# yixuan/LBFGSpp

Measured on AMD Instinct MI355X. Metric: L-BFGS iterations/sec at n=10^8, m=10; achieved HBM GB/s vs peak, higher is better.
Workload: dtype f64; 1 GPU; north-star: extended Rosenbrock n=100000000 m=10 f64 LineSearchMoreThuente, x0 from counter hash; n=100000000, m=10, history_full=True, fevals_total=111, apply_Hv_persistent_launches=82

## Files before the change

include/LBFGS.h:

```cpp
#ifndef LBFGSX_DROPIN_LBFGS_H
#define LBFGSX_DROPIN_LBFGS_H

#include <algorithm>
#include <cmath>
#include <cstdlib>
#include <cstring>
#include <exception>
#include <limits>
#include <stdexcept>
#include <string>
#include <thread>
#include <type_traits>
#include <vector>

#include "LBFGSpp/BKLDLT.h"
#include "LBFGSpp/DenseHessian.h"
#include "LBFGSpp/Device.h"
#include "LBFGSpp/Interop.h"
#include "LBFGSpp/GramSpace.h"
#include "LBFGSpp/LineSearchBacktracking.h"
#include "LBFGSpp/LineSearchBracketing.h"
#include "LBFGSpp/LineSearchMoreThuente.h"
#include "LBFGSpp/LineSearchNocedalWright.h"
#include "LBFGSpp/Param.h"
// ... 78 lines not shown
        if (gram)
        {
            gsh.direction(-1.0, gs_coef, gs_coef_g);
            detail::check(lbfgsx_gs_direction(c, gs_coef.data(), gs_coef_g, &dgd));
            if (m_reducer)
                m_reducer(&dgd, 1);
        }
        else
            detail::check(lbfgsx_apply_Hv(c, LBFGSX_VEC_G, m_dir_scale, &dgd));
        constexpr bool policy_defers =
            detail::takes_pending_dg<LineSearch<Scalar> >::value &&
            detail::has_device_line_search<LineSearch<Scalar>, detail::Evaluator<Scalar, Foo, HostVec>, LBFGSParam<Scalar>, Scalar>::value;
        const bool defer_dg = policy_defers && !gram && !m_reducer && !detail::is_compiled_objective<Scalar, Foo>::value &&
                              ev.builtin_id() >= 0;
        detail::check(lbfgsx_last_in_trial_request(c, defer_dg ? 1 : 0));
        Scalar dg = Scalar(dgd);
        Scalar step = Scalar(1) / m_gnorm;
        constexpr Scalar eps = std::numeric_limits<Scalar>::epsilon();

        int k = 1;
        for (;;)
        {
            detail::Range range_iteration("lbfgs:iteration");
            detail::check(lbfgsx_ls_begin(c));
            if (!gram)
                detail::check(lbfgsx_ls_post_in_trial(c, m_dir_scale));
            const Scalar step_max = m_param.max_step;
            ev.trial_written = false;
            try
            {
// ... 266 lines not shown
```

include/LBFGSpp/Interop.h:

```cpp
#ifndef LBFGSX_DROPIN_INTEROP_H
#define LBFGSX_DROPIN_INTEROP_H

#include <cstdint>
#include <type_traits>
#include <utility>
#include <vector>

#if !defined(LBFGSX_NO_EIGEN) && defined(__has_include)
#if __has_include(<Eigen/Core>)
#include <Eigen/Core>
#define LBFGSX_HAVE_EIGEN 1
#endif
#endif

#include "DenseHessian.h"

namespace LBFGSpp {
namespace detail {

#ifdef LBFGSX_HAVE_EIGEN
template <typename Scalar>
using ResultVector = Eigen::Matrix<Scalar, Eigen::Dynamic, 1>;
template <typename Scalar>
using ResultMatrix = Eigen::Matrix<Scalar, Eigen::Dynamic, Eigen::Dynamic>;
// ... 17 lines not shown

template <typename Policy, typename Ev, typename Param, typename Scalar, typename = void>
struct has_device_line_search : std::false_type {};
template <typename Policy, typename Ev, typename Param, typename Scalar>
struct has_device_line_search<Policy, Ev, Param, Scalar,
                              std::void_t<decltype(Policy::LineSearch(std::declval<Ev&>(), std::declval<const Param&>(),
                                                                      std::declval<const Scalar&>(), std::declval<Scalar&>(),
                                                                      std::declval<Scalar&>(), std::declval<Scalar&>()))> >
    : std::true_type {};

template <typename Policy, typename = void>
struct takes_pending_dg : std::false_type {};
template <typename Policy>
struct takes_pending_dg<Policy, std::enable_if_t<Policy::takes_pending_dg> > : std::true_type {};

template <typename Scalar, typename Ev, typename HostVec>
struct HostObjective
{
    Ev& ev;
    Scalar operator()(const HostVec& x, HostVec& grad) { return ev.eval_host_point(x, grad); }
};

template <typename Scalar, typename Policy, typename HostVec, typename Ev, typename Param>
inline void run_line_search(Ev& ev, const Param& param, const Scalar& step_max, Scalar& step, Scalar& fx, Scalar& dg)
{
    if constexpr (has_device_line_search<Policy, Ev, Param, Scalar>::value)
        Policy::LineSearch(ev, param, step_max, step, fx, dg);
    else
    {
        const std::int64_t n = ev.state().size();
// ... 26 lines not shown
```

include/LBFGSpp/LineSearchMoreThuente.h:

```cpp
#ifndef LBFGSX_DROPIN_LS_MORE_THUENTE_H
#define LBFGSX_DROPIN_LS_MORE_THUENTE_H

#include <algorithm>
#include <cmath>
#include <limits>
#include <stdexcept>

#include "HostEval.h"
#include "Param.h"

namespace LBFGSpp {

template <typename Scalar>
class LineSearchMoreThuente
{
    struct Sample
    {
        Scalar t, f, g;
    };

    static Scalar quad_fgf(const Sample& p, Scalar qt, Scalar fq)
    {
        const Scalar h = qt - p.t;
        const Scalar w = Scalar(0.5) * h * p.g / (p.f - fq + h * p.g);
// ... 206 lines not shown
                }
            }
            m_step = next;
            if (++m_it >= m_max_it)
            {
                m_step = m_lo.t;
                m_fx = m_f_best;
                m_dg = m_g_best;
                return DONE_LO;
            }
            return TRIAL;
        }
    };

    static constexpr bool takes_pending_dg = true;

    template <typename Eval, typename SolverParam>
    static void LineSearch(Eval& ev, const SolverParam& param, const Scalar& step_max, Scalar& step, Scalar& fx,
                           Scalar& dg)
    {
        Machine mt;
        bool have_first = false;
        if constexpr (detail::has_dg_pending<Eval>::value)
        {
            if (ev.dg_pending)
            {
                ev.dg_pending = false;
                mt.start_step(param, step_max, step, fx);
                Scalar f1 = fx, g1 = dg, dg0 = dg;
                have_first = ev.first_trial(mt.step(), f1, g1, dg0);
// ... 46 lines not shown
```

include/lbfgsx.h:

```cpp
#ifndef LBFGSX_H
#define LBFGSX_H

#include <stddef.h>
#include <stdint.h>

#ifdef __cplusplus
extern "C" {
#endif

typedef struct lbfgsx_ctx lbfgsx_ctx;

enum { LBFGSX_F64 = 0, LBFGSX_F32 = 1 };
enum { LBFGSX_OBJ_NONE = -1, LBFGSX_OBJ_DIAG_QUAD = 0, LBFGSX_OBJ_EXT_ROSENBROCK = 1,
       LBFGSX_OBJ_BOUND = 64  };
enum
{
    LBFGSX_OK = 0,
    LBFGSX_E_INVALID = -1,
    LBFGSX_E_LOGIC = -2,
    LBFGSX_E_RUNTIME = -3,
    LBFGSX_E_HIP = -4,
    LBFGSX_E_NOGPU = -5,
    LBFGSX_E_USER = -6
};
// ... 48 lines not shown
int lbfgsx_trial(lbfgsx_ctx* c, int objective, double step, double* fx, double* dg);
int lbfgsx_trial_point(lbfgsx_ctx* c, double step);
int lbfgsx_trial_dg(lbfgsx_ctx* c, double* dg);
int lbfgsx_ls_keep_trial_as_lo(lbfgsx_ctx* c);
int lbfgsx_ls_end(lbfgsx_ctx* c, int use_lo);
int lbfgsx_post_linesearch(lbfgsx_ctx* c, double* gnorm2, double* xnorm2, double* sy, double* yy);
int lbfgsx_commit_correction(lbfgsx_ctx* c);
int lbfgsx_post_linesearch_spec(lbfgsx_ctx* c, double a, double* gnorm2, double* xnorm2, double* sy, double* yy);
int lbfgsx_spec_counts(const lbfgsx_ctx* c, int64_t out[3]);
int lbfgsx_ls_post_in_trial(lbfgsx_ctx* c, double a);
int lbfgsx_post_in_trial_counts(const lbfgsx_ctx* c, int64_t out[4]);
int lbfgsx_last_in_trial_request(lbfgsx_ctx* c, int on);
int lbfgsx_apply_Hv_pending(lbfgsx_ctx* c, int v_which, double a, double* dg, int* pending);
int lbfgsx_trial_first(lbfgsx_ctx* c, int objective, double step, double* fx, double* dg, double* dg_init);
int lbfgsx_last_in_trial_counts(const lbfgsx_ctx* c, int64_t out[4]);
typedef struct lbfgsx_objective lbfgsx_objective;
int lbfgsx_objective_compile(lbfgsx_objective** out, int dtype, int K, const char* body, char* log, size_t log_len);
void lbfgsx_objective_destroy(lbfgsx_objective* obj);
long long lbfgsx_objective_source(int dtype, int K, const char* body, char* out, size_t len);
int lbfgsx_objective_info(const lbfgsx_objective* obj, long long out[8]);
int lbfgsx_objective_K(const lbfgsx_objective* obj);
int lbfgsx_objective_dtype(const lbfgsx_objective* obj);
int lbfgsx_objective_bind(lbfgsx_ctx* c, const lbfgsx_objective* obj, const void* const p[4], const double cs[8], int* id);
int lbfgsx_objective_upload(lbfgsx_ctx* c, int slot, const void* host, void** dev);
int lbfgsx_objective_bound(const lbfgsx_ctx* c, const void* p[4]);
enum { LBFGSX_FORM_TERM = 0, LBFGSX_FORM_CHAIN = 1, LBFGSX_FORM_GRID = 2, LBFGSX_FORM_GRAPH = 3, LBFGSX_FORM_MESH = 4, LBFGSX_FORM_LINEAR = 5,
       LBFGSX_FORM_LINEAR_MULTI = 6, LBFGSX_FORM_DENSE = 7, LBFGSX_FORM_LINEAR_GRAPH = 8, LBFGSX_FORM_VOLUME = 9,
       LBFGSX_FORM_GRID_PERIODIC = 10, LBFGSX_FORM_VOLUME_PERIODIC = 11, LBFGSX_FORM_GRID_FIELD = 12 };
int lbfgsx_objective_compile_chain(lbfgsx_objective** out, int dtype, int K, const char* body, char* log, size_t log_len);
long long lbfgsx_objective_source_chain(int dtype, int K, const char* body, char* out, size_t len);
// ... 277 lines not shown
```

lbfgspp_amd/_lib.py:

```python
import ctypes as C
import os

HERE = os.path.dirname(os.path.abspath(__file__))

F64, F32 = 0, 1
OBJ_DIAG_QUAD, OBJ_EXT_ROSENBROCK = 0, 1
OBJ_BOUND = 64
LS_NOCEDAL_WRIGHT, LS_MORE_THUENTE, LS_BACKTRACKING, LS_BRACKETING = 0, 1, 2, 3
ALGO_LBFGS, ALGO_LBFGSB = 0, 1
RECURSION_VECTOR, RECURSION_GRAM_SPACE, RECURSION_GRAM_SPACE_F32H = 0, 1, 2
FLAG_BOUNDED = 1
(VEC_X, VEC_G, VEC_XP, VEC_GP, VEC_D, VEC_XT, VEC_GT, VEC_A, VEC_B, VEC_LB, VEC_UB, VEC_XCP) = range(12)
E_INVALID, E_LOGIC, E_RUNTIME, E_HIP, E_NOGPU, E_USER = -1, -2, -3, -4, -5, -6


class Params(C.Structure):
    _fields_ = [("m", C.c_int), ("epsilon", C.c_double), ("epsilon_rel", C.c_double), ("past", C.c_int),
                ("delta", C.c_double), ("max_iterations", C.c_int), ("linesearch", C.c_int),
                ("max_linesearch", C.c_int), ("min_step", C.c_double), ("max_step", C.c_double),
                ("ftol", C.c_double), ("wolfe", C.c_double), ("max_submin", C.c_int)]


class Result(C.Structure):
    _fields_ = [("niter", C.c_int), ("nfev", C.c_int), ("fx", C.c_double), ("gnorm", C.c_double),
# ... 85 lines not shown
    sig(core, "lbfgsx_timing_enable", i32, vp, i32)
    sig(core, "lbfgsx_timing_read", i32, vp, pd, C.POINTER(i64), pd, C.POINTER(i64))
    sig(core, "lbfgsx_stream_probe", i32, vp, i32, pd, pd)
    sig(core, "lbfgsx_selftest_reduce", i32, vp, i32, i32, i32, pd)
    sig(core, "lbfgsx_post_linesearch_spec", i32, vp, dbl, pd, pd, pd, pd)
    sig(core, "lbfgsx_rccl_allgather_records", i32, C.POINTER(i32), i32, vp, i64, i64, C.POINTER(vp))
    sig(core, "lbfgsx_device_download", i32, i32, vp, i64, vp)
    sig(core, "lbfgsx_device_free", None, i32, vp)
    sig(core, "lbfgsx_spec_counts", i32, vp, C.POINTER(i64 * 3))
    sig(core, "lbfgsx_ls_post_in_trial", i32, vp, dbl)
    sig(core, "lbfgsx_post_in_trial_counts", i32, vp, C.POINTER(i64 * 4))
    sig(core, "lbfgsx_last_in_trial_request", i32, vp, i32)
    sig(core, "lbfgsx_apply_Hv_pending", i32, vp, i32, dbl, pd, C.POINTER(i32))
    sig(core, "lbfgsx_trial_first", i32, vp, i32, dbl, pd, pd, pd)
    sig(core, "lbfgsx_last_in_trial_counts", i32, vp, C.POINTER(i64 * 4))
    sig(core, "lbfgsx_counters", i32, C.POINTER(i64 * 3), i32)
    sig(core, "lbfgsx_counters_ex", i32, C.POINTER(i64 * 8), i32)
    sig(core, "lbfgsx_poll_counts", i32, vp, C.POINTER(i64 * 2))
    sig(core, "lbfgsx_poll_counts_ex", i32, vp, C.POINTER(i64 * 4))
    sig(core, "lbfgsx_b_compact_vec_counts", i32, C.POINTER(i64 * 4), i32)
    sig(core, "lbfgsx_b_reserve", i32, vp)
    sig(core, "lbfgsx_device", i32, vp)
    sig(core, "lbfgsx_persist_counts", i32, vp, C.POINTER(i64 * 4))
    sig(core, "lbfgsx_debug_persist_fault", i32, vp)

    sig(sol, "lbfgsx_solver_create", i32, C.POINTER(vp), i32, i32, i32, C.POINTER(Params), i32)
    sig(sol, "lbfgsx_solver_create_error", C.c_char_p)
    sig(sol, "lbfgsx_solver_destroy", None, vp)
    sig(sol, "lbfgsx_solver_prepare", i32, vp, i64)
    sig(sol, "lbfgsx_solver_ctx", vp, vp)
# ... 180 lines not shown
```

lbfgspp_amd/csrc/ctx.hpp:

```cpp
#pragma once
#include <hip/hip_runtime.h>
#include <stdint.h>

#include <atomic>
#include <chrono>
#include <string>
#include <vector>

#include "../../include/lbfgsx.h"
#include "last_step.hpp"
#include "reduce.cuh"

struct lbfgsx_ctx;
namespace lbfgsx {

void set_error(const std::string& msg);

#define LBFGSX_HIP(expr)                                                                      \
    do                                                                                        \
    {                                                                                         \
        hipError_t e_ = (expr);                                                               \
        if (e_ != hipSuccess)                                                                 \
        {                                                                                     \
            lbfgsx::set_error(std::string(#expr) + ": " + hipGetErrorString(e_) + " [" + __FILE__ + ":" + std::to_string(__LINE__) + "]");            \
            return LBFGSX_E_HIP;                                                              \
// ... 177 lines not shown
    int spec_cur = 0;
    double spec_a = 0.0, spec_dg = 0.0;
    int64_t spec_launches = 0, spec_used = 0, spec_rejected = 0;
    bool post_in_trial = true;
    bool pt_armed = false;
    double pt_a = 0.0;
    int ls_trials = 0;
    bool ls_first_ok = false;
    bool pt_valid = false;
    int pt_buf = -1, pt_xp = -1;
    double pt_r[4] = {0, 0, 0, 0};
    int64_t pt_issued = 0, pt_accepted = 0;
    int64_t from_g_launches = 0;
    lbfgsx::LastStep last;
    bool pt_builtin = false;

    const struct lbfgsx_objective* term = nullptr;
    void* term_fn[8] = {nullptr, nullptr, nullptr, nullptr, nullptr, nullptr, nullptr, nullptr};
    const void* term_p[4] = {nullptr, nullptr, nullptr, nullptr};
    double term_c[8] = {0, 0, 0, 0, 0, 0, 0, 0};
    int term_np = 0;
    int term_form = 0;
    int64_t term_rows = 0, term_cols = 0;
    int64_t term_slabs = 0;
    int term_periodic = 0;
    void* term_own[4] = {nullptr, nullptr, nullptr, nullptr};
    int64_t term_own_count[4] = {0, 0, 0, 0};
    int64_t graph_E = 0;
    void* graph_off = nullptr;
    void* graph_inc = nullptr;
// ... 121 lines not shown
```

lbfgspp_amd/csrc/lbfgs_kernels.cuh:

```cuda
#pragma once
#include "reduce.cuh"

namespace lbfgsx {

enum { OBJ_DIAG_QUAD = 0, OBJ_EXT_ROSENBROCK = 1 };

template <class T>
struct ObjQuad
{
    const T* a;
    const T* b;
    template <class A>
    __device__ __forceinline__ void pack(int64_t vi, const Pack<T>& x, Pack<T>& g, A& fx) const
    {
        const Pack<T> pa = ldv(a, vi), pb = ldv(b, vi);
#pragma unroll
        for (int k = 0; k < Vec16<T>::W; k++)
        {
            const T r = pa.e[k] * x.e[k] - pb.e[k];
            g.e[k] = pa.e[k] * r;
            fx.add(r * r);
        }
    }
    __device__ __forceinline__ T finish(T sum) const { return T(0.5) * sum; }
// ... 86 lines not shown
    T* dot0;
};

template <class T>
struct TrialLast
{
    const T* snew;
    const T* num;
    const T* num2;
    const T* den;
    T* dot0_keep;
    T* dg_slot;
    T* dout;
};

template <class T, class OBJ, bool POST, bool LAST = false>
__device__ __forceinline__ void trial_pass(const T* __restrict__ xp, const T* __restrict__ d, T step, T* __restrict__ x,
                                           T* __restrict__ g, int64_t n, const OBJ& obj, const RedWs& ws,
                                           T* __restrict__ out, int rev, const TrialPost<T>& tp,
                                           const TrialLast<T>& tl = TrialLast<T>())
{
    typedef typename AccOf<T>::type A;
    constexpr int W = Vec16<T>::W;
    constexpr int U = 4;
    constexpr bool SETTLE = LAST && !POST;
    constexpr int NRED = POST ? (LAST ? 8 : 7) : 2;
    A acc[NRED];
    T coef = T(0);
    if (LAST)
        coef = *tl.num / *tl.den - *tl.num2 / *tl.den;
    const int64_t nv = n / W;
    const int64_t tile = int64_t(kBlock) * U;
    const int64_t top = ((nv + tile - 1) / tile - 1) * tile;
    for (int64_t t0 = int64_t(blockIdx.x) * tile; t0 < nv; t0 += int64_t(gridDim.x) * tile)
    {
        const int64_t base = (rev ? top - t0 : t0) + threadIdx.x;
        Pack<T> pxp[U], pd[U], pgp[POST ? U : 1], psn[LAST ? U : 1];
#pragma unroll
        for (int u = 0; u < U; u++)
            if (base + u * kBlock < nv)
            {
// ... 5 lines not shown
                    pgp[POST ? u : 0] = ldv(tp.gp, base + u * kBlock);
            }
#pragma unroll
        for (int u = 0; u < U; u++)
        {
            const int64_t vi = base + u * kBlock;
            if (vi < nv)
            {
                Pack<T> px, pg;
                if (LAST)
                {
#pragma unroll
                    for (int k = 0; k < W; k++)
                    {
                        pd[u].e[k] = pd[u].e[k] + coef * psn[LAST ? u : 0].e[k];
                        if (POST)
                            acc[POST && LAST ? 7 : 0].add_prod(pgp[POST ? u : 0].e[k], pd[u].e[k]);
                    }
                    if (SETTLE)
                        stv(tl.dout, vi, pd[u]);
                }
#pragma unroll
                for (int k = 0; k < W; k++)
                    px.e[k] = pxp[u].e[k] + step * pd[u].e[k];
                obj.pack(vi, px, pg, acc[0]);
                stv(x, vi, px);
                stv(g, vi, pg);
#pragma unroll
                for (int k = 0; k < W; k++)
                    acc[1].add_prod(pg.e[k], pd[u].e[k]);
                if (POST)
                {
// ... 14 lines not shown
                    stv(tp.y, vi, py);
                }
            }
        }
    }
    if (blockIdx.x == 0 && threadIdx.x == 0)
    {
        auto dir = [&](int64_t i) { return LAST ? d[i] + coef * tl.snew[i] : d[i]; };
        for (int64_t i = nv * W; i < n; i++)
            x[i] = xp[i] + step * dir(i);
        for (int64_t i = nv * W; i < n; i++)
        {
            const T di = dir(i);
            obj.tail(i, n, x, g, acc[0]);
            acc[1].add_prod(g[i], di);
            if (POST && LAST)
                acc[POST && LAST ? 7 : 0].add_prod(tp.gp[i], di);
            if (SETTLE)
                tl.dout[i] = di;
        }
        if (POST)
            for (int64_t i = nv * W; i < n; i++)
            {
                const T si = x[i] - xp[i], yi = g[i] - tp.gp[i], q0 = tp.a * g[i];
                tp.s[i] = si;
                tp.y[i] = yi;
                acc[POST ? 2 : 0].add_prod(g[i], g[i]);
                acc[POST ? 3 : 0].add_prod(x[i], x[i]);
                acc[POST ? 4 : 0].add_prod(si, yi);
                acc[POST ? 5 : 0].add_prod(yi, yi);
                acc[POST ? 6 : 0].add_prod(si, q0);
            }
    }
    if (grid_reduce<NRED>(acc, ws) && threadIdx.x == 0)
    {
        out[0] = obj.finish(T(acc[0].value()));
        out[1] = T(acc[1].value());
        if (POST)
        {
            const T sy = T(acc[POST ? 4 : 0].value()), yy = T(acc[POST ? 5 : 0].value());
            out[2] = T(acc[POST ? 2 : 0].value());
            out[3] = T(acc[POST ? 3 : 0].value());
            out[4] = sy;
            out[5] = yy;
            if (LAST)
            {
                const T dgd = T(acc[LAST ? 7 : 0].value());
                out[6] = dgd;
                *tl.dg_slot = dgd;
                *tl.dot0_keep = *tl.num;
            }
            *tp.ys_slot = sy;
            *tp.theta_slot = yy / sy;
            *tp.dot0 = T(acc[POST ? 6 : 0].value());
        }
        ws_signal(ws);
    }
}

template <class T, class OBJ>
__global__ void __launch_bounds__(kBlock) k_trial(const T* __restrict__ xp, const T* __restrict__ d, T step,
                                                  T* __restrict__ x, T* __restrict__ g, int64_t n, OBJ obj,
// ... 10 lines not shown
}
template <class T, class OBJ>
__global__ void __launch_bounds__(kBlock, 4) k_trial_last(const T* __restrict__ xp, const T* __restrict__ q, T step,
                                                       T* __restrict__ x, T* __restrict__ g, int64_t n, OBJ obj,
                                                       RedWs ws, T* __restrict__ out, int rev, TrialPost<T> tp,
                                                       TrialLast<T> tl)
{
    trial_pass<T, OBJ, true, true>(xp, q, step, x, g, n, obj, ws, out, rev, tp, tl);
}
template <class T, class OBJ>
__global__ void __launch_bounds__(kBlock) k_trial_settle(const T* __restrict__ xp, const T* q, T step, T* __restrict__ x,
                                                         T* __restrict__ g, int64_t n, OBJ obj, RedWs ws,
                                                         T* __restrict__ out, int rev, TrialLast<T> tl)
{
    trial_pass<T, OBJ, false, true>(xp, q, step, x, g, n, obj, ws, out, rev, TrialPost<T>(), tl);
}

template <class T>
__global__ void __launch_bounds__(kBlock) k_axpy_point(const T* __restrict__ xp, const T* __restrict__ d, T step,
                                                       T* __restrict__ x, int64_t n)
{
    constexpr int W = Vec16<T>::W;
    const int64_t nv = n / W;
    const int64_t stride = int64_t(gridDim.x) * kBlock;
    for (int64_t vi = int64_t(blockIdx.x) * kBlock + threadIdx.x; vi < nv; vi += stride)
    {
        const Pack<T> pxp = ldv(xp, vi), pd = ldv(d, vi);
        Pack<T> px;
#pragma unroll
        for (int k = 0; k < W; k++)
// ... 968 lines not shown
```

lbfgspp_amd/csrc/lbfgsx.hip:

```cpp
#include <dlfcn.h>

#include <algorithm>
#include <atomic>
#include <cmath>
#include <chrono>
#include <string>
#include <vector>
#include <utility>
#include <cstdio>
#include <cstdlib>
#include <cstring>
#include <limits>
#include <mutex>

#include "ctx.hpp"
#include "lbfgs_kernels.cuh"
#include "launch_args.hpp"

namespace lbfgsx {

static std::atomic<int> g_live[64];
Counters& counters()
{
    static Counters g;
// ... 365 lines not shown
        if (n < min_n)
            c->persist = false;
    }
    if (const char* e = getenv("LBFGSX_PERSIST"))
        c->persist = atoi(e) != 0 && c->persist;
    if (const char* e = getenv("LBFGSX_MEET"))
        c->meet_all = std::strcmp(e, "last") != 0;
    if (const char* e = getenv("LBFGSX_PERSIST_POLL"))
        c->fast_persist_out = atoi(e) != 0;
    if (const char* e = getenv("LBFGSX_FUSE_POST"))
        c->fuse_post = atoi(e) != 0;
    if (const char* e = getenv("LBFGSX_POST_IN_TRIAL"))
        c->post_in_trial = atoi(e) != 0;
    if (const char* e = getenv("LBFGSX_LAST_IN_TRIAL"))
        c->last.enabled = atoi(e) != 0;
    {
        int occ = 0;
        hipDeviceProp_t prop;
        LBFGSX_HIP(hipGetDeviceProperties(&prop, device));
        if (dtype == LBFGSX_F64)
            (void) hipOccupancyMaxActiveBlocksPerMultiprocessor(&occ, k_twoloop_persist<double, true, true>, kHvThreads, 0);
        else
            (void) hipOccupancyMaxActiveBlocksPerMultiprocessor(&occ, k_twoloop_persist<float, true, true>, kHvThreads, 0);
        c->persist_grid = occ * prop.multiProcessorCount;
        c->gen_words = 16 + size_t(10) * size_t(c->persist_grid) * 4;
        LBFGSX_HIP(hipMalloc(reinterpret_cast<void**>(&c->gen_dev), c->gen_words * sizeof(unsigned)));
        LBFGSX_HIP(hipMemset(c->gen_dev, 0, c->gen_words * sizeof(unsigned)));
    }
    const size_t vbytes = size_t(c->ld) * c->esz;
    for (int k = 0; k < 3; k++)
// ... 660 lines not shown
        const T* g = P<T>(c->gb[c->cur]);
        LBFGSX_LAUNCH((k_dot<T>), dim3(grid), dim3(kBlock), 0, c->stream, g, g, P<T>(c->xb[c->cur]), c->n, c->ws,
                           c->out_slot<T>());
        int rc = fetch_scalars<T>(c, c->sl.out(0), 2, r);
        if (rc)
            return rc;
    });
    if (gnorm2) *gnorm2 = r[0];
    if (xnorm2) *xnorm2 = r[1];
    return LBFGSX_OK;
}

int lbfgsx_ls_begin(lbfgsx_ctx* c)
{
    c->st_valid = false;
    c->pt_valid = c->pt_armed = false;
    c->ls_trials = 0;
    c->xp = c->cur;
    c->lo = c->xp;
    c->trial = (c->xp + 1) % 3;
    return LBFGSX_OK;
}

}
template <class T, class OBJ>
static int trial_t(lbfgsx_ctx* c, OBJ obj, T step, double* out2)
{
    const lbfgsx::TrialLaunch<T> a = lbfgsx::trial_launch<T>(c, step, sizeof(OBJ) >= 2 * sizeof(void*) ? 2 : 0);
    LBFGSX_LAUNCH((k_trial<T, OBJ>), dim3(a.grid), dim3(kBlock), 0, c->stream, a.xp, a.d, a.step, a.x, a.g, a.n, obj, a.ws,
                       a.out, a.rev);
    LBFGSX_HIP(hipGetLastError());
    return fetch_scalars<T>(c, c->sl.out(0), 2, out2);
}
template <class T>
static lbfgsx::TrialPost<T> trial_post_args(lbfgsx_ctx* c)
{
    T* sc = P<T>(c->sc);
    return {P<T>(c->gb[c->xp]), P<T>(c->col(c->S, c->spare)), P<T>(c->col(c->Y, c->spare)), T(c->pt_a),
            sc + c->sl.ys(c->spare), sc + c->sl.theta(c->spare), sc + c->sl.dot(0)};
}
static void trial_post_done(lbfgsx_ctx* c, const double* out6)
{
    c->pending = false;
    c->pt_valid = true;
    c->pt_buf = c->trial;
    c->pt_xp = c->xp;
    for (int i = 0; i < 4; i++)
        c->pt_r[i] = out6[2 + i];
    c->pt_issued++;
}
template <class T, class OBJ>
static int trial_post_t(lbfgsx_ctx* c, OBJ obj, T step, double* out2)
{
    const lbfgsx::TrialLaunch<T> a = lbfgsx::trial_launch<T>(c, step, sizeof(OBJ) >= 2 * sizeof(void*) ? 2 : 0);
    const lbfgsx::TrialPost<T> tp = trial_post_args<T>(c);
    LBFGSX_LAUNCH((k_trial_post<T, OBJ>), dim3(a.grid), dim3(kBlock), 0, c->stream, a.xp, a.d, a.step, a.x, a.g, a.n, obj,
                       a.ws, a.out, a.rev, tp);
    LBFGSX_HIP(hipGetLastError());
    double r[6];
    const int rc = fetch_scalars<T>(c, c->sl.out(0), 6, r);
    if (rc)
        return rc;
    out2[0] = r[0];
    out2[1] = r[1];
    trial_post_done(c, r);
    c->pt_builtin = true;
    return LBFGSX_OK;
}
template <class T, class OBJ>
static int trial_last_t(lbfgsx_ctx* c, OBJ obj, T step, double* out3)
{
    const lbfgsx::LastStep& ls = c->last;
    if (ls.col == c->spare)
    {
        set_error("lbfgsx_trial: the newest history column is the spare column");
        return LBFGSX_E_LOGIC;
    }
    c->tl_step++;
    const lbfgsx::TrialLaunch<T> a = lbfgsx::trial_launch<T>(c, step, (sizeof(OBJ) >= 2 * sizeof(void*) ? 2 : 0) + 1);
    const lbfgsx::TrialPost<T> tp = trial_post_args<T>(c);
// ... 29 lines not shown
    T* sc = P<T>(c->sc);
    const lbfgsx::TrialLast<T> tl = {static_cast<const T*>(c->col(c->S, ls.col)), sc + c->sl.dot(2 * c->m + 1),
                                     sc + c->sl.dot(2 * ls.cn - 1), sc + c->sl.ys(ls.col), nullptr, nullptr, P<T>(c->d)};
    EventPair ev;
    int rc = last_time_begin(c, ev);
    if (rc)
        return rc;
    LBFGSX_LAUNCH((k_trial_settle<T, OBJ>), dim3(a.grid), dim3(kBlock), 0, c->stream, a.xp, a.d, a.step, a.x, a.g, a.n, obj,
                       a.ws, a.out, a.rev, tl);
    LBFGSX_HIP(hipGetLastError());
    if ((rc = last_time_end(c, ev)))
        return rc;
    (void) c->last.settle([](const lbfgsx::LastStep&) { return 0; });
    return fetch_scalars<T>(c, c->sl.out(0), 2, out2);
}
template <class T>
static int trial_post_term_t(lbfgsx_ctx* c, T step, double* out2)
{
    lbfgsx::TrialLaunch<T> a = lbfgsx::trial_launch<T>(c, step, c->term_np);
    lbfgsx::BoundArgs<T> obj(c);
    lbfgsx::TrialPost<T> tp = trial_post_args<T>(c);
    void* params[] = {&a.xp, &a.d, &a.step, &a.x, &a.g, &a.n, obj.ptr, &a.ws, &a.out, &a.rev, &tp};
    int rc = lbfgsx::jit_launch(c, lbfgsx::JIT_K_TRIAL_POST, a.grid, params);
    if (rc)
        return rc;
    double r[6];
    rc = fetch_scalars<T>(c, c->sl.out(0), 6, r);
    if (rc)
        return rc;
    out2[0] = r[0];
    out2[1] = r[1];
    trial_post_done(c, r);
    c->pt_builtin = false;
    return LBFGSX_OK;
}
template <class T>
static int trial_term_t(lbfgsx_ctx* c, T step, double* out2)
{
    lbfgsx::TrialLaunch<T> a = lbfgsx::trial_launch<T>(c, step, c->term_np);
    lbfgsx::BoundArgs<T> obj(c);
    lbfgsx::objective_model_add<T>(c, 2);
    void* params[] = {&a.xp, &a.d, &a.step, &a.x, &a.g, &a.n, obj.ptr, &a.ws, &a.out, &a.rev};
    int rc = lbfgsx::linear_pre_trial<T>(c, obj, a.xp, a.d, a.step);
    if (rc)
        return rc;
    rc = lbfgsx::jit_launch(c, lbfgsx::JIT_K_TRIAL, lbfgsx::linear_col_grid(c, a.grid), params);
    if (rc)
// ... 2 lines not shown
}
extern "C" {

int lbfgsx_trial(lbfgsx_ctx* c, int objective, double step, double* fx, double* dg)
{
    return lbfgsx_trial_first(c, objective, step, fx, dg, nullptr);
}

int lbfgsx_trial_first(lbfgsx_ctx* c, int objective, double step, double* fx, double* dg, double* dg_init)
{
    lbfgsx::DeviceGuard dev_guard_(c->device);
    c->spec_valid = false;
    double r[3];
    int rc = LBFGSX_E_INVALID;
    const bool builtin = objective == LBFGSX_OBJ_DIAG_QUAD || objective == LBFGSX_OBJ_EXT_ROSENBROCK;
    const bool last = c->last.fusable(c->pt_armed && c->ls_trials == 0, builtin, dg_init != nullptr, c->xp) && !c->st_valid;
    const int last_cn = c->last.cn;
    const bool settle_here = !last && c->last.pending && c->last.taken && builtin && !c->st_valid && c->xp == c->last.g;
    if (!last && !settle_here)
        LBFGSX_SETTLE(c);
    const bool owed = c->last.pay() && dg_init && !last;
    if (dg_init)
        *dg_init = std::numeric_limits<double>::quiet_NaN();
    if (c->st_valid)
    {
        c->st_valid = false;
        bool same = objective == c->st_obj && c->xp == c->st_xp && c->trial == c->st_trial;
        DISPATCH_T(c, { same = same && T(step) == T(c->st_step); });
        if (same)
        {
            c->st_hits++;
            c->ls_trials++;
            c->tl_step++;
            if (fx) *fx = c->st_f;
            if (dg) *dg = c->st_dg;
            return LBFGSX_OK;
        }
        c->st_cooldown = 4;
    }
    const bool post = c->pt_armed && c->ls_trials == 0 &&
                      (objective == LBFGSX_OBJ_DIAG_QUAD || objective == LBFGSX_OBJ_EXT_ROSENBROCK ||
                       (lbfgsx::term_bound(c, objective) && c->term_fn[lbfgsx::JIT_K_TRIAL_POST] != nullptr));
    c->ls_trials++;
    c->pt_valid = false;
    DISPATCH_T(c, {
        if (objective == LBFGSX_OBJ_DIAG_QUAD)
            rc = last          ? trial_last_t<T>(c, ObjQuad<T>{P<T>(c->a), P<T>(c->b)}, T(step), r)
                 : settle_here ? trial_settle_t<T>(c, ObjQuad<T>{P<T>(c->a), P<T>(c->b)}, T(step), r)
                 : post        ? trial_post_t<T>(c, ObjQuad<T>{P<T>(c->a), P<T>(c->b)}, T(step), r)
                               : trial_t<T>(c, ObjQuad<T>{P<T>(c->a), P<T>(c->b)}, T(step), r);
        else if (objective == LBFGSX_OBJ_EXT_ROSENBROCK)
            rc = last          ? trial_last_t<T>(c, ObjRosen<T>{}, T(step), r)
                 : settle_here ? trial_settle_t<T>(c, ObjRosen<T>{}, T(step), r)
                 : post        ? trial_post_t<T>(c, ObjRosen<T>{}, T(step), r)
                               : trial_t<T>(c, ObjRosen<T>{}, T(step), r);
        else if (lbfgsx::term_bound(c, objective))
            rc = post ? trial_post_term_t<T>(c, T(step), r) : trial_term_t<T>(c, T(step), r);
        else
            set_error("lbfgsx_trial: unknown objective");
        if (!rc && owed)
            rc = fetch_scalars<T>(c, c->sl.dot(2 * last_cn), 1, dg_init);
    });
    if (rc)
        return rc;
    if (fx) *fx = r[0];
    if (dg) *dg = r[1];
    if (last) *dg_init = r[2];
    return LBFGSX_OK;
}

int lbfgsx_trial_point(lbfgsx_ctx* c, double step)
{
// ... 203 lines not shown
        LBFGSX_HIP(hipMemsetAsync(c->ws.ticket, 0, sizeof(unsigned), c->stream));
        c->gen_count = 0;
        persist_timed_out(c);
        if (c->timing && !c->ev_hv.empty())
        {
            (void) hipEventDestroy(c->ev_hv.back().a);
            (void) hipEventDestroy(c->ev_hv.back().b);
            c->ev_hv.pop_back();
            c->persist_steps_timed -= 2 * cn + 1;
            c->fused_timed -= fused;
        }
        return 1;
    }
    c->persist_launches++;
    c->spec_launches++;
    c->from_g_launches += from_g ? 1 : 0;
    c->persist_backoff = 8;
    if (hflags[1] == 1)
    {
        c->spec_valid = true;
        c->spec_version = c->phys_version + 1;
        c->spec_cur = c->cur;
        c->spec_a = double(a);
        c->spec_dg = dgv;
        if (defer)
        {
            c->spec_dg = std::numeric_limits<double>::quiet_NaN();
            c->last.defer(cn, pa.pcol[0], c->cur);
        }
    }
    else
// ... 11 lines not shown
    return LBFGSX_OK;
}
extern "C" {

int lbfgsx_post_linesearch_spec(lbfgsx_ctx* c, double a, double* gnorm2, double* xnorm2, double* sy, double* yy)
{
    lbfgsx::DeviceGuard dev_guard_(c->device);
    if (c->gs_f32h)
        return lbfgsx_post_linesearch(c, gnorm2, xnorm2, sy, yy);
    double r[4];
    int rc = 1;
    c->spec_valid = false;
    if (c->pt_valid && c->cur == c->pt_buf && c->xp == c->pt_xp)
    {
        c->pt_valid = false;
        c->pt_accepted++;
        for (int i = 0; i < 4; i++)
            r[i] = c->pt_r[i];
        c->pend_sy = r[2];
        c->pend_yy = r[3];
        c->pending = true;
        bool usable = false;
        DISPATCH_T(c, { usable = a == c->pt_a && T(r[2]) > std::numeric_limits<T>::epsilon() * T(r[3]); });
        if (usable)
        {
            DISPATCH_T(c, { rc = post_spec_t<T>(c, T(a), r, true); });
            if (rc != LBFGSX_OK && rc != 1)
                return rc;
        }
        if (gnorm2) *gnorm2 = r[0];
        if (xnorm2) *xnorm2 = r[1];
// ... 12 lines not shown
    c->pending = true;
    if (gnorm2) *gnorm2 = r[0];
    if (xnorm2) *xnorm2 = r[1];
    if (sy) *sy = r[2];
    if (yy) *yy = r[3];
    return LBFGSX_OK;
}

int lbfgsx_ls_post_in_trial(lbfgsx_ctx* c, double a)
{
    if (!c)
        return LBFGSX_E_INVALID;
    c->pt_a = a;
    c->pt_armed = c->post_in_trial && c->ls_first_ok && c->ncorr > 0 && !c->gs_f32h && c->ls_trials == 0 &&
                  c->shard_off == 0 && c->n_global == c->n;
    return LBFGSX_OK;
}

int lbfgsx_post_in_trial_counts(const lbfgsx_ctx* c, int64_t out[4])
{
    if (!c || !out)
        return LBFGSX_E_INVALID;
    out[0] = c->pt_issued;
    out[1] = c->pt_accepted;
    out[2] = c->from_g_launches;
    out[3] = c->post_in_trial ? 1 : 0;
    return LBFGSX_OK;
}

int lbfgsx_last_in_trial_request(lbfgsx_ctx* c, int on)
{
    if (!c)
        return LBFGSX_E_INVALID;
    c->last.requested = on != 0 && !c->bstate;
    return LBFGSX_OK;
}

int lbfgsx_last_in_trial_counts(const lbfgsx_ctx* c, int64_t out[4])
{
    if (!c || !out)
        return LBFGSX_E_INVALID;
// ... 326 lines not shown
```

Measured before the change: 92.76 iterations/s.

## Fuse post-linesearch reductions into second and third line-search trials

Extends the post-in-trial fusion, which computes the post-linesearch reductions (sy, yy, norms) inside the trial kernel, from the first trial to trials 2 and 3 of More-Thuente. It adds a combined settle+post trial kernel and a small decision function that picks the trial form. The goal is to skip a separate full-vector post pass when the line search accepts a later trial. In exchange, non-accepted later trials do extra reduction work, and the trial-state logic gets more complex.

Measured after the change: 93.37 iterations/s (median of 5 runs). About the same (+0.7%).

```diff
diff --git a/include/LBFGS.h b/include/LBFGS.h
--- a/include/LBFGS.h
+++ b/include/LBFGS.h
@@ -116,6 +116,10 @@
         const bool defer_dg = policy_defers && !gram && !m_reducer && !detail::is_compiled_objective<Scalar, Foo>::value &&
                               ev.builtin_id() >= 0;
         detail::check(lbfgsx_last_in_trial_request(c, defer_dg ? 1 : 0));
+        constexpr bool policy_posts_later =
+            detail::posts_later_trials<LineSearch<Scalar> >::value &&
+            detail::has_device_line_search<LineSearch<Scalar>, detail::Evaluator<Scalar, Foo, HostVec>, LBFGSParam<Scalar>, Scalar>::value;
+        detail::check(lbfgsx_post_in_later_trials_request(c, policy_posts_later && !gram && !m_reducer ? 1 : 0));
         Scalar dg = Scalar(dgd);
         Scalar step = Scalar(1) / m_gnorm;
         constexpr Scalar eps = std::numeric_limits<Scalar>::epsilon();
diff --git a/include/LBFGSpp/Interop.h b/include/LBFGSpp/Interop.h
--- a/include/LBFGSpp/Interop.h
+++ b/include/LBFGSpp/Interop.h
@@ -55,6 +55,11 @@
 template <typename Policy>
 struct takes_pending_dg<Policy, std::enable_if_t<Policy::takes_pending_dg> > : std::true_type {};
 
+template <typename Policy, typename = void>
+struct posts_later_trials : std::false_type {};
+template <typename Policy>
+struct posts_later_trials<Policy, std::enable_if_t<Policy::posts_later_trials> > : std::true_type {};
+
 template <typename Scalar, typename Ev, typename HostVec>
 struct HostObjective
 {
diff --git a/include/LBFGSpp/LineSearchMoreThuente.h b/include/LBFGSpp/LineSearchMoreThuente.h
--- a/include/LBFGSpp/LineSearchMoreThuente.h
+++ b/include/LBFGSpp/LineSearchMoreThuente.h
@@ -244,6 +244,7 @@
     };
 
     static constexpr bool takes_pending_dg = true;
+    static constexpr bool posts_later_trials = true;
 
     template <typename Eval, typename SolverParam>
     static void LineSearch(Eval& ev, const SolverParam& param, const Scalar& step_max, Scalar& step, Scalar& fx,
diff --git a/include/lbfgsx.h b/include/lbfgsx.h
--- a/include/lbfgsx.h
+++ b/include/lbfgsx.h
@@ -86,6 +86,8 @@
 int lbfgsx_apply_Hv_pending(lbfgsx_ctx* c, int v_which, double a, double* dg, int* pending);
 int lbfgsx_trial_first(lbfgsx_ctx* c, int objective, double step, double* fx, double* dg, double* dg_init);
 int lbfgsx_last_in_trial_counts(const lbfgsx_ctx* c, int64_t out[4]);
+int lbfgsx_post_in_later_trials_request(lbfgsx_ctx* c, int on);
+int lbfgsx_post_in_later_trials_counts(const lbfgsx_ctx* c, int64_t out[4]);
 typedef struct lbfgsx_objective lbfgsx_objective;
 int lbfgsx_objective_compile(lbfgsx_objective** out, int dtype, int K, const char* body, char* log, size_t log_len);
 void lbfgsx_objective_destroy(lbfgsx_objective* obj);
diff --git a/lbfgspp_amd/_lib.py b/lbfgspp_amd/_lib.py
--- a/lbfgspp_amd/_lib.py
+++ b/lbfgspp_amd/_lib.py
@@ -123,6 +123,8 @@
     sig(core, "lbfgsx_apply_Hv_pending", i32, vp, i32, dbl, pd, C.POINTER(i32))
     sig(core, "lbfgsx_trial_first", i32, vp, i32, dbl, pd, pd, pd)
     sig(core, "lbfgsx_last_in_trial_counts", i32, vp, C.POINTER(i64 * 4))
+    sig(core, "lbfgsx_post_in_later_trials_request", i32, vp, i32)
+    sig(core, "lbfgsx_post_in_later_trials_counts", i32, vp, C.POINTER(i64 * 4))
     sig(core, "lbfgsx_counters", i32, C.POINTER(i64 * 3), i32)
     sig(core, "lbfgsx_counters_ex", i32, C.POINTER(i64 * 8), i32)
     sig(core, "lbfgsx_poll_counts", i32, vp, C.POINTER(i64 * 2))
diff --git a/lbfgspp_amd/csrc/ctx.hpp b/lbfgspp_amd/csrc/ctx.hpp
--- a/lbfgspp_amd/csrc/ctx.hpp
+++ b/lbfgspp_amd/csrc/ctx.hpp
@@ -9,6 +9,7 @@
 
 #include "../../include/lbfgsx.h"
 #include "last_step.hpp"
+#include "trial_form.hpp"
 #include "reduce.cuh"
 
 struct lbfgsx_ctx;
@@ -216,6 +217,11 @@
     int64_t from_g_launches = 0;
     lbfgsx::LastStep last;
     bool pt_builtin = false;
+    bool post_later = true;
+    bool pl_requested = false;
+    bool pl_armed = false;
+    bool pt_later = false;
+    int64_t pl_issued = 0, pl_accepted = 0, pl_from_g = 0, pl_settle_post = 0;
 
     const struct lbfgsx_objective* term = nullptr;
     void* term_fn[8] = {nullptr, nullptr, nullptr, nullptr, nullptr, nullptr, nullptr, nullptr};
diff --git a/lbfgspp_amd/csrc/lbfgs_kernels.cuh b/lbfgspp_amd/csrc/lbfgs_kernels.cuh
--- a/lbfgspp_amd/csrc/lbfgs_kernels.cuh
+++ b/lbfgspp_amd/csrc/lbfgs_kernels.cuh
@@ -124,7 +124,7 @@
     T* dout;
 };
 
-template <class T, class OBJ, bool POST, bool LAST = false>
+template <class T, class OBJ, bool POST, bool LAST = false, bool SETTLE = LAST && !POST>
 __device__ __forceinline__ void trial_pass(const T* __restrict__ xp, const T* __restrict__ d, T step, T* __restrict__ x,
                                            T* __restrict__ g, int64_t n, const OBJ& obj, const RedWs& ws,
                                            T* __restrict__ out, int rev, const TrialPost<T>& tp,
@@ -133,8 +133,8 @@
     typedef typename AccOf<T>::type A;
     constexpr int W = Vec16<T>::W;
     constexpr int U = 4;
-    constexpr bool SETTLE = LAST && !POST;
-    constexpr int NRED = POST ? (LAST ? 8 : 7) : 2;
+    constexpr bool DGD = POST && LAST && !SETTLE;
+    constexpr int NRED = POST ? (DGD ? 8 : 7) : 2;
     A acc[NRED];
     T coef = T(0);
     if (LAST)
@@ -170,8 +170,8 @@
                     for (int k = 0; k < W; k++)
                     {
                         pd[u].e[k] = pd[u].e[k] + coef * psn[LAST ? u : 0].e[k];
-                        if (POST)
-                            acc[POST && LAST ? 7 : 0].add_prod(pgp[POST ? u : 0].e[k], pd[u].e[k]);
+                        if (DGD)
+                            acc[DGD ? 7 : 0].add_prod(pgp[POST ? u : 0].e[k], pd[u].e[k]);
                     }
                     if (SETTLE)
                         stv(tl.dout, vi, pd[u]);
@@ -216,8 +216,8 @@
             const T di = dir(i);
             obj.tail(i, n, x, g, acc[0]);
             acc[1].add_prod(g[i], di);
-            if (POST && LAST)
-                acc[POST && LAST ? 7 : 0].add_prod(tp.gp[i], di);
+            if (DGD)
+                acc[DGD ? 7 : 0].add_prod(tp.gp[i], di);
             if (SETTLE)
                 tl.dout[i] = di;
         }
@@ -245,9 +245,9 @@
             out[3] = T(acc[POST ? 3 : 0].value());
             out[4] = sy;
             out[5] = yy;
-            if (LAST)
-            {
-                const T dgd = T(acc[LAST ? 7 : 0].value());
+            if (DGD)
+            {
+                const T dgd = T(acc[DGD ? 7 : 0].value());
                 out[6] = dgd;
                 *tl.dg_slot = dgd;
                 *tl.dot0_keep = *tl.num;
@@ -288,6 +288,14 @@
                                                          T* __restrict__ out, int rev, TrialLast<T> tl)
 {
     trial_pass<T, OBJ, false, true>(xp, q, step, x, g, n, obj, ws, out, rev, TrialPost<T>(), tl);
+}
+template <class T, class OBJ>
+__global__ void __launch_bounds__(kBlock, 4) k_trial_settle_post(const T* __restrict__ xp, const T* q, T step,
+                                                                 T* __restrict__ x, T* __restrict__ g, int64_t n, OBJ obj,
+                                                                 RedWs ws, T* __restrict__ out, int rev, TrialPost<T> tp,
+                                                                 TrialLast<T> tl)
+{
+    trial_pass<T, OBJ, true, true, true>(xp, q, step, x, g, n, obj, ws, out, rev, tp, tl);
 }
 
 template <class T>
diff --git a/lbfgspp_amd/csrc/lbfgsx.hip b/lbfgspp_amd/csrc/lbfgsx.hip
--- a/lbfgspp_amd/csrc/lbfgsx.hip
+++ b/lbfgspp_amd/csrc/lbfgsx.hip
@@ -403,6 +403,8 @@
         c->post_in_trial = atoi(e) != 0;
     if (const char* e = getenv("LBFGSX_LAST_IN_TRIAL"))
         c->last.enabled = atoi(e) != 0;
+    if (const char* e = getenv("LBFGSX_POST_IN_LATER_TRIALS"))
+        c->post_later = atoi(e) != 0;
     {
         int occ = 0;
         hipDeviceProp_t prop;
@@ -1093,7 +1095,7 @@
 int lbfgsx_ls_begin(lbfgsx_ctx* c)
 {
     c->st_valid = false;
-    c->pt_valid = c->pt_armed = false;
+    c->pt_valid = c->pt_armed = c->pl_armed = false;
     c->ls_trials = 0;
     c->xp = c->cur;
     c->lo = c->xp;
@@ -1118,7 +1120,7 @@
     return {P<T>(c->gb[c->xp]), P<T>(c->col(c->S, c->spare)), P<T>(c->col(c->Y, c->spare)), T(c->pt_a),
             sc + c->sl.ys(c->spare), sc + c->sl.theta(c->spare), sc + c->sl.dot(0)};
 }
-static void trial_post_done(lbfgsx_ctx* c, const double* out6)
+static void trial_post_done(lbfgsx_ctx* c, const double* out6, bool later = false)
 {
     c->pending = false;
     c->pt_valid = true;
@@ -1126,10 +1128,11 @@
     c->pt_xp = c->xp;
     for (int i = 0; i < 4; i++)
         c->pt_r[i] = out6[2 + i];
-    c->pt_issued++;
+    c->pt_later = later;
+    (later ? c->pl_issued : c->pt_issued)++;
 }
 template <class T, class OBJ>
-static int trial_post_t(lbfgsx_ctx* c, OBJ obj, T step, double* out2)
+static int trial_post_t(lbfgsx_ctx* c, OBJ obj, T step, double* out2, bool later)
 {
     const lbfgsx::TrialLaunch<T> a = lbfgsx::trial_launch<T>(c, step, sizeof(OBJ) >= 2 * sizeof(void*) ? 2 : 0);
     const lbfgsx::TrialPost<T> tp = trial_post_args<T>(c);
@@ -1142,7 +1145,7 @@
         return rc;
     out2[0] = r[0];
     out2[1] = r[1];
-    trial_post_done(c, r);
+    trial_post_done(c, r, later);
     c->pt_builtin = true;
     return LBFGSX_OK;
 }
@@ -1202,8 +1205,43 @@
     (void) c->last.settle([](const lbfgsx::LastStep&) { return 0; });
     return fetch_scalars<T>(c, c->sl.out(0), 2, out2);
 }
+template <class T, class OBJ>
+static int trial_settle_post_t(lbfgsx_ctx* c, OBJ obj, T step, double* out2)
+{
+    const lbfgsx::LastStep& ls = c->last;
+    if (ls.col == c->spare)
+    {
+        set_error("lbfgsx_trial: the newest history column is the spare column");
+        return LBFGSX_E_LOGIC;
+    }
+    const lbfgsx::TrialLaunch<T> a = lbfgsx::trial_launch<T>(c, step, (sizeof(OBJ) >= 2 * sizeof(void*) ? 2 : 0) + 2);
+    const lbfgsx::TrialPost<T> tp = trial_post_args<T>(c);
+    T* sc = P<T>(c->sc);
+    const lbfgsx::TrialLast<T> tl = {static_cast<const T*>(c->col(c->S, ls.col)), sc + c->sl.dot(2 * c->m + 1),
+                                     sc + c->sl.dot(2 * ls.cn - 1), sc + c->sl.ys(ls.col), nullptr, nullptr, P<T>(c->d)};
+    EventPair ev;
+    int rc = last_time_begin(c, ev);
+    if (rc)
+        return rc;
+    LBFGSX_LAUNCH((k_trial_settle_post<T, OBJ>), dim3(a.grid), dim3(kBlock), 0, c->stream, a.xp, a.d, a.step, a.x, a.g, a.n,
+                       obj, a.ws, a.out, a.rev, tp, tl);
+    LBFGSX_HIP(hipGetLastError());
+    if ((rc = last_time_end(c, ev)))
+        return rc;
+    (void) c->last.settle([](const lbfgsx::LastStep&) { return 0; });
+    double r[6];
+    rc = fetch_scalars<T>(c, c->sl.out(0), 6, r);
+    if (rc)
+        return rc;
+    out2[0] = r[0];
+    out2[1] = r[1];
+    trial_post_done(c, r, true);
+    c->pt_builtin = true;
+    c->pl_settle_post++;
+    return LBFGSX_OK;
+}
 template <class T>
-static int trial_post_term_t(lbfgsx_ctx* c, T step, double* out2)
+static int trial_post_term_t(lbfgsx_ctx* c, T step, double* out2, bool later)
 {
     lbfgsx::TrialLaunch<T> a = lbfgsx::trial_launch<T>(c, step, c->term_np);
     lbfgsx::BoundArgs<T> obj(c);
@@ -1218,7 +1256,7 @@
         return rc;
     out2[0] = r[0];
     out2[1] = r[1];
-    trial_post_done(c, r);
+    trial_post_done(c, r, later);
     c->pt_builtin = false;
     return LBFGSX_OK;
 }
@@ -1251,10 +1289,21 @@
     double r[3];
     int rc = LBFGSX_E_INVALID;
     const bool builtin = objective == LBFGSX_OBJ_DIAG_QUAD || objective == LBFGSX_OBJ_EXT_ROSENBROCK;
-    const bool last = c->last.fusable(c->pt_armed && c->ls_trials == 0, builtin, dg_init != nullptr, c->xp) && !c->st_valid;
+    const lbfgsx::TrialStep step_state =
+        c->st_valid || !c->last.pending || c->xp != c->last.g ? lbfgsx::TRIAL_STEP_NONE
+        : c->last.taken                                       ? lbfgsx::TRIAL_STEP_TAKEN
+        : dg_init != nullptr                                  ? lbfgsx::TRIAL_STEP_OWED
+                                                              : lbfgsx::TRIAL_STEP_NONE;
+    const lbfgsx::TrialObjective kind =
+        builtin ? lbfgsx::TRIAL_OBJ_BUILTIN
+        : lbfgsx::term_bound(c, objective) && c->term_fn[lbfgsx::JIT_K_TRIAL_POST] != nullptr ? lbfgsx::TRIAL_OBJ_TERM_POST
+                                                                                                 : lbfgsx::TRIAL_OBJ_OTHER;
+    const lbfgsx::TrialForm form = lbfgsx::trial_form(c->pt_armed, c->pl_armed, c->ls_trials + 1, step_state, kind);
+    const bool last = form == lbfgsx::TRIAL_LAST;
+    const bool settle_here = form == lbfgsx::TRIAL_SETTLE, settle_post = form == lbfgsx::TRIAL_SETTLE_POST;
+    const bool post = form == lbfgsx::TRIAL_POST, later = c->ls_trials > 0;
     const int last_cn = c->last.cn;
-    const bool settle_here = !last && c->last.pending && c->last.taken && builtin && !c->st_valid && c->xp == c->last.g;
-    if (!last && !settle_here)
+    if (!last && !settle_here && !settle_post)
         LBFGSX_SETTLE(c);
     const bool owed = c->last.pay() && dg_init && !last;
     if (dg_init)
@@ -1275,24 +1324,23 @@
         }
         c->st_cooldown = 4;
     }
-    const bool post = c->pt_armed && c->ls_trials == 0 &&
-                      (objective == LBFGSX_OBJ_DIAG_QUAD || objective == LBFGSX_OBJ_EXT_ROSENBROCK ||
-                       (lbfgsx::term_bound(c, objective) && c->term_fn[lbfgsx::JIT_K_TRIAL_POST] != nullptr));
     c->ls_trials++;
     c->pt_valid = false;
     DISPATCH_T(c, {
         if (objective == LBFGSX_OBJ_DIAG_QUAD)
             rc = last          ? trial_last_t<T>(c, ObjQuad<T>{P<T>(c->a), P<T>(c->b)}, T(step), r)
                  : settle_here ? trial_settle_t<T>(c, ObjQuad<T>{P<T>(c->a), P<T>(c->b)}, T(step), r)
-                 : post        ? trial_post_t<T>(c, ObjQuad<T>{P<T>(c->a), P<T>(c->b)}, T(step), r)
+                 : settle_post ? trial_settle_post_t<T>(c, ObjQuad<T>{P<T>(c->a), P<T>(c->b)}, T(step), r)
+                 : post        ? trial_post_t<T>(c, ObjQuad<T>{P<T>(c->a), P<T>(c->b)}, T(step), r, later)
                                : trial_t<T>(c, ObjQuad<T>{P<T>(c->a), P<T>(c->b)}, T(step), r);
         else if (objective == LBFGSX_OBJ_EXT_ROSENBROCK)
             rc = last          ? trial_last_t<T>(c, ObjRosen<T>{}, T(step), r)
                  : settle_here ? trial_settle_t<T>(c, ObjRosen<T>{}, T(step), r)
-                 : post        ? trial_post_t<T>(c, ObjRosen<T>{}, T(step), r)
+                 : settle_post ? trial_settle_post_t<T>(c, ObjRosen<T>{}, T(step), r)
+                 : post        ? trial_post_t<T>(c, ObjRosen<T>{}, T(step), r, later)
                                : trial_t<T>(c, ObjRosen<T>{}, T(step), r);
         else if (lbfgsx::term_bound(c, objective))
-            rc = post ? trial_post_term_t<T>(c, T(step), r) : trial_term_t<T>(c, T(step), r);
+            rc = post ? trial_post_term_t<T>(c, T(step), r, later) : trial_term_t<T>(c, T(step), r);
         else
             set_error("lbfgsx_trial: unknown objective");
         if (!rc && owed)
@@ -1526,7 +1574,8 @@
     }
     c->persist_launches++;
     c->spec_launches++;
-    c->from_g_launches += from_g ? 1 : 0;
+    if (from_g)
+        (c->pt_later ? c->pl_from_g : c->from_g_launches)++;
     c->persist_backoff = 8;
     if (hflags[1] == 1)
     {
@@ -1568,7 +1617,7 @@
     if (c->pt_valid && c->cur == c->pt_buf && c->xp == c->pt_xp)
     {
         c->pt_valid = false;
-        c->pt_accepted++;
+        (c->pt_later ? c->pl_accepted : c->pt_accepted)++;
         for (int i = 0; i < 4; i++)
             r[i] = c->pt_r[i];
         c->pend_sy = r[2];
@@ -1611,6 +1660,8 @@
     c->pt_a = a;
     c->pt_armed = c->post_in_trial && c->ls_first_ok && c->ncorr > 0 && !c->gs_f32h && c->ls_trials == 0 &&
                   c->shard_off == 0 && c->n_global == c->n;
+    c->pl_armed = c->post_in_trial && c->post_later && c->pl_requested && c->ncorr > 0 && !c->gs_f32h && c->ls_trials == 0 &&
+                  c->shard_off == 0 && c->n_global == c->n;
     return LBFGSX_OK;
 }
 
@@ -1622,6 +1673,25 @@
     out[1] = c->pt_accepted;
     out[2] = c->from_g_launches;
     out[3] = c->post_in_trial ? 1 : 0;
+    return LBFGSX_OK;
+}
+
+int lbfgsx_post_in_later_trials_request(lbfgsx_ctx* c, int on)
+{
+    if (!c)
+        return LBFGSX_E_INVALID;
+    c->pl_requested = on != 0 && !c->bstate;
+    return LBFGSX_OK;
+}
+
+int lbfgsx_post_in_later_trials_counts(const lbfgsx_ctx* c, int64_t out[4])
+{
+    if (!c || !out)
+        return LBFGSX_E_INVALID;
+    out[0] = c->pl_issued;
+    out[1] = c->pl_accepted;
+    out[2] = c->pl_from_g;
+    out[3] = c->pl_settle_post;
     return LBFGSX_OK;
 }
 
diff --git a/lbfgspp_amd/csrc/trial_form.hpp b/lbfgspp_amd/csrc/trial_form.hpp
--- /dev/null
+++ b/lbfgspp_amd/csrc/trial_form.hpp
@@ -0,0 +1,35 @@
+#pragma once
+
+namespace lbfgsx {
+
+enum TrialForm { TRIAL_PLAIN = 0, TRIAL_POST = 1, TRIAL_LAST = 2, TRIAL_SETTLE = 3, TRIAL_SETTLE_POST = 4 };
+
+enum TrialObjective
+{
+    TRIAL_OBJ_BUILTIN = 0,
+    TRIAL_OBJ_TERM_POST = 1,
+    TRIAL_OBJ_OTHER = 2
+};
+
+enum TrialStep
+{
+    TRIAL_STEP_NONE = 0,
+    TRIAL_STEP_OWED = 1,
+    TRIAL_STEP_TAKEN = 2
+};
+
+enum { kLaterPostFirst = 2, kLaterPostLast = 3 };
+
+inline TrialForm trial_form(bool first_armed, bool later_armed, int trial, TrialStep step, TrialObjective obj)
+{
+    const bool has_post = obj == TRIAL_OBJ_BUILTIN || obj == TRIAL_OBJ_TERM_POST;
+    const bool post_first = first_armed && trial == 1 && has_post;
+    const bool post_later = later_armed && trial >= kLaterPostFirst && trial <= kLaterPostLast && has_post;
+    if (step == TRIAL_STEP_OWED && post_first && obj == TRIAL_OBJ_BUILTIN)
+        return TRIAL_LAST;
+    if (step == TRIAL_STEP_TAKEN && obj == TRIAL_OBJ_BUILTIN)
+        return post_later ? TRIAL_SETTLE_POST : TRIAL_SETTLE;
+    return post_first || post_later ? TRIAL_POST : TRIAL_PLAIN;
+}
+
+}
```
